# dayae1204/WeCLIP-ViT-CoMer

Measured on AMD Instinct MI355X. Metric: images/sec (train fwd+bwd) ViT-B/16 512x512 VOC, higher is better.
Workload: dtype f16 MFMA operands / f32 accumulate, f32 residual+softmax+LN, PAR f32 arithmetic on 16-bit fixed-point affinities (precision=fast); 1 GPU; WeCLIP VOC full train step (the reference's model: frozen CLIP ViT-B/16 + adapters + decoder + GradCAM/affinity/PAR pseudo-labels), batch 16/GPU at 512x512, K=2 classes/image (BASELINE configs[2] without the ViT-CoMer inserts, for which the reference has no code); global_batch=16, parallelism=dp1

## Files before the change

weclip-vit-comer_amd/csrc/affinity.hip:

```cpp
#include "common.h"

#define MAXK 4

struct MapPtrs {
    const float* p[12];
};

__global__ __launch_bounds__(256) void aff_weight_kernel(MapPtrs maps, int nmaps, const float* __restrict__ wgt,
                                                          const float* __restrict__ seg, float* __restrict__ W,
                                                          int L) {
    const int hw = L - 1;
    const int j = blockIdx.x * 256 + threadIdx.x, i = blockIdx.y, b = blockIdx.z;
    if (j >= hw) return;
    const long src = (long)b * L * L + (long)(i + 1) * L + (j + 1);
    float v[12];
#pragma unroll
    for (int l = 0; l < 12; ++l) v[l] = l < nmaps ? maps.p[l][src] : 0.f;
    float s = 0.f;
#pragma unroll
    for (int l = 0; l < 12; ++l)
        if (l < nmaps) s = fmaf(wgt[b * nmaps + l], v[l], s);
    const long dst = ((long)b * hw + i) * hw + j;
    if (seg) s *= seg[dst];
    W[dst] = s;
// ... 249 lines not shown
                    a += w[r][ch].x * cx[ch][0][k] + w[r][ch].y * cx[ch][1][k] + w[r][ch].z * cx[ch][2][k] + w[r][ch].w * cx[ch][3][k];
                p[r][k] = wave_sum(a);
            }
        if (lane == 0) {
#pragma unroll
            for (int r = 0; r < AF_RG; ++r)
#pragma unroll
                for (int k = 0; k < K; ++k) red[buf][wave][r][k] = p[r][k];
        }
        __syncthreads();
#pragma unroll
        for (int r = 0; r < AF_RG; ++r) {
            const int i = ig + r;
            if (i >= i1) continue;
            float rv[K];
#pragma unroll
            for (int k = 0; k < K; ++k) {
                const float dot = red[buf][0][r][k] + red[buf][1][r][k] + red[buf][2][r][k] + red[buf][3][r][k];
                if (MODE == 2) {
                    const float ri = rix[r];
                    if (tid == 0) y1[((long)b * hw + i) * K + k] = ri * dot;
                    rv[k] = ri * xix[r][k];
                } else {
                    rv[k] = 1.0f / dot;
                    if (tid == 0) rout[(long)b * hw + i] = rv[k];
                }
            }
            if (MODE != 1) {
#pragma unroll
                for (int ch = 0; ch < AF_MAXCH; ++ch)
#pragma unroll
                    for (int k = 0; k < K; ++k) {
                        ca[ch][0][k] = fmaf(w[r][ch].x, rv[k], ca[ch][0][k]);
                        ca[ch][1][k] = fmaf(w[r][ch].y, rv[k], ca[ch][1][k]);
                        ca[ch][2][k] = fmaf(w[r][ch].z, rv[k], ca[ch][2][k]);
                        ca[ch][3][k] = fmaf(w[r][ch].w, rv[k], ca[ch][3][k]);
                    }
            }
        }
    }
    if (MODE != 1) {
#pragma unroll
        for (int ch = 0; ch < AF_MAXCH; ++ch) {
            if (!okc[ch]) continue;
            const int j = ch * 1024 + tid * 4;
#pragma unroll
            for (int q = 0; q < 4; ++q)
#pragma unroll
                for (int k = 0; k < K; ++k) colpart[(((long)b * nblk + blk) * hw + j + q) * K + k] = ca[ch][q][k];
        }
    }
}

__global__ __launch_bounds__(256) void aff_colreduce_kernel(const float* __restrict__ colpart, const float* __restrict__ y1,
                                                             const float* __restrict__ c, float* __restrict__ out, int hw,
                                                             int K, int nblk, int mode) {
    const int e = blockIdx.x * 256 + threadIdx.x, b = blockIdx.y;
    if (e >= hw * K) return;
    const float* cp = colpart + (long)b * nblk * hw * K + e;
    const long st = (long)hw * K;
    float s = 0.f;
    int blk = 0;
    for (; blk + 8 <= nblk; blk += 8) {
        float v[8];
#pragma unroll
        for (int u = 0; u < 8; ++u) v[u] = cp[(blk + u) * st];
        s += ((v[0] + v[1]) + (v[2] + v[3])) + ((v[4] + v[5]) + (v[6] + v[7]));
    }
    for (; blk < nblk; ++blk) s += cp[blk * st];
    if (mode == 0) out[(long)b * hw + e] = 1.0f / s;
    else out[(long)b * hw * K + e] = 0.5f * (y1[(long)b * hw * K + e] + c[(long)b * hw + e / K] * s);
}

__global__ __launch_bounds__(256) void tsym_kernel(const float* __restrict__ W, const float* __restrict__ r,
                                                    const float* __restrict__ c, float* __restrict__ T, int hw) {
    const int j = blockIdx.x * 256 + threadIdx.x, i = blockIdx.y, b = blockIdx.z;
    if (j >= hw) return;
    const float* Wb = W + (long)b * hw * hw;
    const float* rb = r + (long)b * hw;
    const float* cb = c + (long)b * hw;
    T[((long)b * hw + i) * hw + j] = 0.5f * (rb[i] * Wb[(long)i * hw + j] * cb[j] + cb[i] * Wb[(long)j * hw + i] * rb[j]);
}

__global__ __launch_bounds__(256) void box_mask_kernel(const float* __restrict__ cam, const int* __restrict__ pair_img,
                                                        const int* __restrict__ pair_slot, float* __restrict__ V,
                                                        float* __restrict__ mask_out, int* __restrict__ boxes,
                                                        int* __restrict__ nbox, int maxbox, int h, int w, int K,
                                                        double thr) {
    extern __shared__ int smi[];
    const int hw = h * w, p = blockIdx.x, tid = threadIdx.x;
    int* lab = smi;
    int* xmin = lab + hw;
    int* xmax = xmin + hw;
    int* ymin = xmax + hw;
    int* ymax = ymin + hw;
    int* roots = ymax + hw;
    int* misc = roots + hw;
    const float* cp = cam + (long)p * hw;
    if (tid == 0) { misc[0] = 0; misc[2] = 0; }
    __syncthreads();
    int mx = 0;
    for (int i = tid; i < hw; i += 256) {
        const int u = (int)(unsigned char)(cp[i] * 255.0f);
        mx = u > mx ? u : mx;
    }
    atomicMax(&misc[0], mx);
    __syncthreads();
    const int theta = (int)(thr * (double)misc[0]);
    for (int i = tid; i < hw; i += 256) {
        const int u = (int)(unsigned char)(cp[i] * 255.0f);
        lab[i] = (u > theta) ? i : -1;
        xmin[i] = w; xmax[i] = -1; ymin[i] = h; ymax[i] = -1;
    }
    __syncthreads();
    for (int it = 0; it < hw + 2; ++it) {
        if (tid == 0) misc[1] = 0;
        __syncthreads();
        int changed = 0;
        for (int i = tid; i < hw; i += 256) {
            int l = lab[i];
            if (l < 0) continue;
            const int y = i / w, x = i - y * w;
            int best = l;
            for (int dy = -1; dy <= 1; ++dy)
                for (int dx = -1; dx <= 1; ++dx) {
                    const int yy = y + dy, xx = x + dx;
                    if (yy < 0 || yy >= h || xx < 0 || xx >= w) continue;
                    const int nl = lab[yy * w + xx];
                    if (nl >= 0 && nl < best) best = nl;
                }
            if (best < l) { lab[i] = best; changed = 1; }
        }
        if (changed) misc[1] = 1;
        __syncthreads();
        if (misc[1] == 0) break;
        for (int i = tid; i < hw; i += 256) {
            const int l = lab[i];
            if (l >= 0) {
                const int ll = lab[l];
                if (ll < l) lab[i] = ll;
            }
        }
        __syncthreads();
    }
    for (int i = tid; i < hw; i += 256) {
        int l = lab[i];
        if (l < 0) continue;
        while (lab[l] != l) l = lab[l];
        const int y = i / w, x = i - y * w;
        atomicMin(&xmin[l], x); atomicMax(&xmax[l], x);
        atomicMin(&ymin[l], y); atomicMax(&ymax[l], y);
    }
    __syncthreads();
    for (int i = tid; i < hw; i += 256)
        if (lab[i] == i) roots[atomicAdd(&misc[2], 1)] = i;
    __syncthreads();
    const int nroot = misc[2];
    if (boxes) {
        if (tid == 0) nbox[p] = nroot;
        for (int k = tid; k < nroot && k < maxbox; k += 256) {
            const int r = roots[k];
            int* bx = boxes + ((long)p * maxbox + k) * 4;
            bx[0] = xmin[r]; bx[1] = ymin[r];
            bx[2] = (xmax[r] + 1 < w - 1) ? xmax[r] + 1 : w - 1;
            bx[3] = (ymax[r] + 1 < h - 1) ? ymax[r] + 1 : h - 1;
        }
    }
    const int img = pair_img[p], slot = pair_slot[p];
    for (int i = tid; i < hw; i += 256) {
        const int y = i / w, x = i - y * w;
        int inside = 0;
        for (int k = 0; k < nroot && !inside; ++k) {
            const int r = roots[k];
            const int x0 = xmin[r], y0 = ymin[r];
            int x1 = xmax[r] + 1, y1 = ymax[r] + 1;
            x1 = x1 < w - 1 ? x1 : w - 1;
            y1 = y1 < h - 1 ? y1 : h - 1;
            inside = (x >= x0 && x < x1 && y >= y0 && y < y1);
        }
        if (mask_out) mask_out[(long)p * hw + i] = inside ? 1.f : 0.f;
        if (slot >= 0) V[((long)img * hw + i) * K + slot] = inside ? cp[i] : 0.f;
    }
}

__global__ __launch_bounds__(256) void refined_minmax_kernel(const float* __restrict__ R, float* __restrict__ stats,
                                                              int hw, int K) {
    __shared__ float red[16];
    const int k = blockIdx.x, b = blockIdx.y;
    float mn = INFINITY, mx = -INFINITY;
    for (int i = threadIdx.x; i < hw; i += 256) {
        const float v = R[((long)b * hw + i) * K + k];
        mn = fminf(mn, v);
        mx = fmaxf(mx, v);
    }
    mn = block_min(mn, red);
    mx = block_max(mx, red);
    if (threadIdx.x == 0) {
        stats[((long)b * K + k) * 2] = mn;
        stats[((long)b * K + k) * 2 + 1] = mx - mn;
    }
}

__global__ __launch_bounds__(256) void cam_upsample_kernel(const float* __restrict__ R, const float* __restrict__ stats,
                                                            const int* __restrict__ nk, float* __restrict__ cams,
                                                            int h, int w, int K, int C, int H, int W, float sy, float sx) {
    const int x = blockIdx.x * 64 + (threadIdx.x & 63), y = blockIdx.y * 4 + (threadIdx.x >> 6), b = blockIdx.z;
    if (x >= W || y >= H) return;
    float fy = fmaxf(sy * (y + 0.5f) - 0.5f, 0.f), fx = fmaxf(sx * (x + 0.5f) - 0.5f, 0.f);
    int y0 = (int)fy, x0 = (int)fx;
    if (y0 > h - 1) y0 = h - 1;
    if (x0 > w - 1) x0 = w - 1;
    const int y1 = y0 + (y0 < h - 1 ? 1 : 0), x1 = x0 + (x0 < w - 1 ? 1 : 0);
    const float ly = fy - y0, lx = fx - x0, hy = 1.f - ly, hx = 1.f - lx;
    const long HW = (long)H * W;
    const int n = nk[b];
    float best = -INFINITY;
    const float* Rb = R + (long)b * h * w * K;
    for (int k = 0; k < n; ++k) {
        const float mn = stats[((long)b * K + k) * 2], den = 1e-7f + stats[((long)b * K + k) * 2 + 1];
        const float v00 = (Rb[((long)y0 * w + x0) * K + k] - mn) / den, v01 = (Rb[((long)y0 * w + x1) * K + k] - mn) / den;
        const float v10 = (Rb[((long)y1 * w + x0) * K + k] - mn) / den, v11 = (Rb[((long)y1 * w + x1) * K + k] - mn) / den;
        const float v = hy * (hx * v00 + lx * v01) + ly * (hx * v10 + lx * v11);
        cams[((long)b * C + 1 + k) * HW + (long)y * W + x] = v;
        best = fmaxf(best, v);
    }
    for (int k = n; k < C - 1; ++k) cams[((long)b * C + 1 + k) * HW + (long)y * W + x] = 0.f;
    cams[(long)b * C * HW + (long)y * W + x] = 1.0f - best;
}

extern "C" int wc_aff_weight(const float* const* h_maps, int nmaps, const float* wgt, const float* seg, float* W,
                             int B, int L, void* stream) {
    WC_CHECK_ARG(h_maps && nmaps >= 1 && nmaps <= 12 && wgt && W && B > 0 && L > 1, "wc_aff_weight: bad argument");
    MapPtrs mp;
    for (int i = 0; i < 12; ++i) mp.p[i] = i < nmaps ? h_maps[i] : nullptr;
    const int hw = L - 1;
    hipLaunchKernelGGL(aff_weight_kernel, dim3(wc_cdiv(hw, 256), hw, B), dim3(256), 0, (hipStream_t)stream, mp, nmaps,
                       wgt, seg, W, L);
    WC_LAUNCH_CHECK("aff_weight_kernel");
    return WC_OK;
}

extern "C" int wc_aff_seg_weights(const float* const* h_maps, int nmaps, float* rowsum, float* diff, float* wgt,
                                  int B, int L, void* stream) {
    WC_CHECK_ARG(h_maps && nmaps >= 1 && nmaps <= 12 && rowsum && diff && wgt && B > 0 && L > 1,
                 "wc_aff_seg_weights: bad argument");
    MapPtrs mp;
    for (int i = 0; i < 12; ++i) mp.p[i] = i < nmaps ? h_maps[i] : nullptr;
    hipStream_t st = (hipStream_t)stream;
    hipLaunchKernelGGL(aff_rowsum_kernel, dim3(L - 1, nmaps, B), dim3(256), 0, st, mp, nmaps, rowsum, L);
    WC_LAUNCH_CHECK("aff_rowsum_kernel");
    hipLaunchKernelGGL(aff_keep_kernel, dim3(B), dim3(64), 0, st, rowsum, diff, wgt, nmaps, L - 1);
    WC_LAUNCH_CHECK("aff_keep_kernel");
    return WC_OK;
}

extern "C" int wc_matvec(const float* W, const float* X, const float* sin, const float* sout, const float* add,
                         float* out, int B, int hw, int K, int transpose, int recip, float alpha, void* stream) {
    WC_CHECK_ARG(W && X && out && B > 0 && hw > 0 && K > 0 && B <= 65535, "wc_matvec: bad argument");
    WC_CHECK_ARG(out != X && out != sin, "wc_matvec: out must not alias an input vector");
    hipStream_t st = (hipStream_t)stream;
    for (int k0 = 0; k0 < K; k0 += MAXK) {
        if (transpose)
            hipLaunchKernelGGL(matvec_cols_kernel, dim3(wc_cdiv(hw, 64), B), dim3(64 * MVC_SLICES), 0, st, W, X, sin, sout, add,
                               out, hw, K, k0, recip, alpha);
        else
            hipLaunchKernelGGL(matvec_rows_kernel, dim3(wc_cdiv(hw, 4), B), dim3(256), 0, st, W, X, sin, sout, add,
                               out, hw, K, k0, recip, alpha);
        WC_LAUNCH_CHECK("matvec kernel");
    }
    return WC_OK;
}

static bool aff_fused_ok(int hw) { return hw % 4 == 0 && hw <= 1024 * AF_MAXCH && hw >= 4; }

extern "C" int wc_aff_fused_supported(int hw) { return aff_fused_ok(hw) ? 1 : 0; }

extern "C" int wc_aff_weight_c1(const float* const* h_maps, int nmaps, const float* wgt, const float* seg, float* W, float* c1,
                                float* ws, int B, int L, void* stream) {
    WC_CHECK_ARG(h_maps && nmaps >= 1 && nmaps <= 12 && wgt && W && c1 && ws && B > 0 && B <= 65535 && L > 1 && aff_fused_ok(L - 1),
                 "wc_aff_weight_c1: bad argument");
    MapPtrs mp;
    for (int i = 0; i < 12; ++i) mp.p[i] = i < nmaps ? h_maps[i] : nullptr;
    const int hw = L - 1, nblk = wc_cdiv(hw, AF_RPBW);
    hipStream_t st = (hipStream_t)stream;
    const int pr = wc_prof_begin(stream);
    hipLaunchKernelGGL(aff_weight_colpart_kernel, dim3(nblk, B), dim3(256), 0, st, mp, nmaps, wgt, seg, W, ws, L);
    wc_prof_end(pr, "aff_weight_colpart_kernel", (double)B * hw * hw * 4.0 * (nmaps + 1 + (seg ? 1 : 0)), stream);
    WC_LAUNCH_CHECK("aff_weight_colpart_kernel");
    hipLaunchKernelGGL(aff_colreduce_kernel, dim3(wc_cdiv(hw, 256), B), dim3(256), 0, st, ws, nullptr, nullptr, c1, hw, 1, nblk, 0);
    WC_LAUNCH_CHECK("aff_colreduce_kernel");
    return WC_OK;
}

extern "C" int wc_aff_sinkhorn_step(const float* W, const float* c, float* r, float* c_next, float* ws, int B, int hw,
                                    int last, void* stream) {
    WC_CHECK_ARG(W && c && r && ws && (last || c_next) && B > 0 && B <= 65535 && aff_fused_ok(hw), "wc_aff_sinkhorn_step: bad argument");
    const int nblk = wc_cdiv(hw, AF_RPB);
    hipStream_t st = (hipStream_t)stream;
    const int pr = wc_prof_begin(stream);
    if (last) hipLaunchKernelGGL((aff_sweep_kernel<1, 1>), dim3(nblk, B), dim3(256), 0, st, W, c, nullptr, nullptr, r, nullptr, ws, hw);
    else hipLaunchKernelGGL((aff_sweep_kernel<0, 1>), dim3(nblk, B), dim3(256), 0, st, W, c, nullptr, nullptr, r, nullptr, ws, hw);
    wc_prof_end(pr, "aff_sweep_kernel", (double)B * hw * hw * 4.0 * (last ? 1 : 2), stream);
    WC_LAUNCH_CHECK("aff_sweep_kernel");
    if (!last) {
        hipLaunchKernelGGL(aff_colreduce_kernel, dim3(wc_cdiv(hw, 256), B), dim3(256), 0, st, ws, nullptr, nullptr, c_next, hw, 1, nblk, 0);
        WC_LAUNCH_CHECK("aff_colreduce_kernel");
    }
    return WC_OK;
}

extern "C" int wc_aff_tsym_apply(const float* W, const float* r, const float* c, const float* X, float* out, float* y1,
                                 float* ws, int B, int hw, int K, void* stream) {
    WC_CHECK_ARG(W && r && c && X && out && y1 && ws && out != X && B > 0 && B <= 65535 && K >= 1 && K <= 4 && aff_fused_ok(hw),
                 "wc_aff_tsym_apply: bad argument (K <= 4)");
    const int nblk = wc_cdiv(hw, AF_RPB);
    hipStream_t st = (hipStream_t)stream;
    dim3 grid(nblk, B);
    const int pr = wc_prof_begin(stream);
    switch (K) {
        case 1: hipLaunchKernelGGL((aff_sweep_kernel<2, 1>), grid, dim3(256), 0, st, W, c, r, X, nullptr, y1, ws, hw); break;
        case 2: hipLaunchKernelGGL((aff_sweep_kernel<2, 2>), grid, dim3(256), 0, st, W, c, r, X, nullptr, y1, ws, hw); break;
        case 3: hipLaunchKernelGGL((aff_sweep_kernel<2, 3>), grid, dim3(256), 0, st, W, c, r, X, nullptr, y1, ws, hw); break;
        default: hipLaunchKernelGGL((aff_sweep_kernel<2, 4>), grid, dim3(256), 0, st, W, c, r, X, nullptr, y1, ws, hw); break;
    }
    wc_prof_end(pr, "aff_sweep_kernel", (double)B * hw * hw * 4.0 * 2, stream);
    WC_LAUNCH_CHECK("aff_sweep_kernel");
    hipLaunchKernelGGL(aff_colreduce_kernel, dim3(wc_cdiv(hw * K, 256), B), dim3(256), 0, st, ws, y1, c, out, hw, K, nblk, 1);
    WC_LAUNCH_CHECK("aff_colreduce_kernel");
    return WC_OK;
}

extern "C" int wc_tsym(const float* W, const float* r, const float* c, float* T, int B, int hw, void* stream) {
    WC_CHECK_ARG(W && r && c && T && B > 0 && hw > 0, "wc_tsym: bad argument");
    hipLaunchKernelGGL(tsym_kernel, dim3(wc_cdiv(hw, 256), hw, B), dim3(256), 0, (hipStream_t)stream, W, r, c, T, hw);
    WC_LAUNCH_CHECK("tsym_kernel");
    return WC_OK;
}

extern "C" int wc_box_mask(const float* cam, const int* pair_img, const int* pair_slot, float* V, float* mask_out,
                           int* boxes, int* nbox, int maxbox, int P, int h, int w, int K, double thr, void* stream) {
    WC_CHECK_ARG(cam && pair_img && pair_slot && V && P > 0 && h > 0 && w > 0 && K > 0, "wc_box_mask: bad argument");
    WC_CHECK_ARG(!boxes || (nbox && maxbox > 0), "wc_box_mask: boxes needs nbox and maxbox");
    const size_t sm = ((size_t)6 * h * w + 4) * sizeof(int);
    WC_CHECK_ARG(sm <= 160 * 1024, "wc_box_mask: CAM grid too large (h*w <= 6800)");
    hipLaunchKernelGGL(box_mask_kernel, dim3(P), dim3(256), sm, (hipStream_t)stream, cam, pair_img, pair_slot, V,
                       mask_out, boxes, nbox, maxbox, h, w, K, thr);
    WC_LAUNCH_CHECK("box_mask_kernel");
    return WC_OK;
}

extern "C" int wc_cam_upsample(const float* R, const int* nk, float* stats, float* cams, int B, int h, int w, int K,
                               int C, int H, int W, void* stream) {
    WC_CHECK_ARG(R && nk && stats && cams && B > 0 && h > 0 && w > 0 && K > 0 && C >= 2 && C <= K + 1 && H > 0 && W > 0,
                 "wc_cam_upsample: bad argument");
    hipStream_t st = (hipStream_t)stream;
    hipLaunchKernelGGL(refined_minmax_kernel, dim3(K, B), dim3(256), 0, st, R, stats, h * w, K);
    WC_LAUNCH_CHECK("refined_minmax_kernel");
    hipLaunchKernelGGL(cam_upsample_kernel, dim3(wc_cdiv(W, 64), wc_cdiv(H, 4), B), dim3(256), 0, st, R, stats, nk,
                       cams, h, w, K, C, H, W, (float)h / H, (float)w / W);
    WC_LAUNCH_CHECK("cam_upsample_kernel");
    return WC_OK;
}
```

weclip-vit-comer_amd/csrc/gradcam.hip:

```cpp
#include "common.h"

typedef _Float16 f16x8 __attribute__((ext_vector_type(8)));
typedef float f32x16 __attribute__((ext_vector_type(16)));

#define LNP_ROWS 16
template <int NV>
__global__ __launch_bounds__(256) void lnpost_pool_kernel(const float* __restrict__ x2,
                                                           const float* __restrict__ w,
                                                           const float* __restrict__ bb, float eps,
                                                           float* __restrict__ partial, int L, int E,
                                                           int nchunk) {
    extern __shared__ float sm[];
    const int b = blockIdx.y, chunk = blockIdx.x, lane = threadIdx.x & 63, wv = threadIdx.x >> 6;
    float acc[NV], wv_[NV], bv[NV];
#pragma unroll
    for (int i = 0; i < NV; ++i) {
        const int e = lane + 64 * i;
        acc[i] = 0.f;
        wv_[i] = e < E ? w[e] : 0.f;
        bv[i] = e < E ? bb[e] : 0.f;
    }
    const int l0 = chunk * LNP_ROWS;
    for (int l = l0 + wv; l < l0 + LNP_ROWS && l < L; l += 4) {
        if (l == 0) continue;
        const float* xr = x2 + ((long)b * L + l) * E;
        float xv[NV];
        float s = 0.f;
#pragma unroll
        for (int i = 0; i < NV; ++i) {
            const int e = lane + 64 * i;
            xv[i] = e < E ? xr[e] : 0.f;
            s += xv[i];
        }
        const float mean = wave_sum(s) / E;
        float q = 0.f;
#pragma unroll
        for (int i = 0; i < NV; ++i) {
            const float d = (lane + 64 * i < E) ? xv[i] - mean : 0.f;
            q += d * d;
        }
        const float rstd = rsqrtf(wave_sum(q) / E + eps);
#pragma unroll
        for (int i = 0; i < NV; ++i)
            if (lane + 64 * i < E) acc[i] += (xv[i] - mean) * rstd * wv_[i] + bv[i];
    }
#pragma unroll
    for (int i = 0; i < NV; ++i)
        if (lane + 64 * i < E) sm[wv * E + lane + 64 * i] = acc[i];
    __syncthreads();
    for (int e = threadIdx.x; e < E; e += 256)
        partial[((long)b * nchunk + chunk) * E + e] = sm[e] + sm[E + e] + sm[2 * E + e] + sm[3 * E + e];
}

__global__ __launch_bounds__(512) void cam_head_kernel(const float* __restrict__ partial,
                                                        const float* __restrict__ proj,
                                                        const float* __restrict__ text,
                                                        const int* __restrict__ text_idx,
                                                        const int* __restrict__ n_text,
                                                        const int* __restrict__ pair_img,
                                                        const int* __restrict__ pair_cls, float logit_scale,
                                                        float* __restrict__ probs, float* __restrict__ df,
                                                        int L, int E, int Ed, int nchunk, int Tmax) {
    extern __shared__ float sm[];
    float* f = sm;
    float* y = f + E;
    float* dy = y + Ed;
    float* lg = dy + Ed;
    float* red = lg + Tmax;
    const int p = blockIdx.x, img = pair_img[p], cls = pair_cls[p], T = n_text[p], tid = threadIdx.x;
    for (int e = tid; e < E; e += 512) {
        const float* pp = partial + (long)img * nchunk * E + e;
        float s[8] = {0.f, 0.f, 0.f, 0.f, 0.f, 0.f, 0.f, 0.f};
        int c = 0;
        for (; c + 8 <= nchunk; c += 8)
#pragma unroll
            for (int u = 0; u < 8; ++u) s[u] += pp[(long)(c + u) * E];
        for (; c < nchunk; ++c) s[0] += pp[(long)c * E];
        f[e] = (((s[0] + s[1]) + (s[2] + s[3])) + ((s[4] + s[5]) + (s[6] + s[7]))) / (L - 1);
    }
    __syncthreads();
    for (int t = tid; t < Ed; t += 512) {
        float s0 = 0.f, s1 = 0.f, s2 = 0.f, s3 = 0.f;
        int e = 0;
        for (; e + 16 <= E; e += 16) {
            float pv[16];
#pragma unroll
            for (int u = 0; u < 16; ++u) pv[u] = proj[(long)(e + u) * Ed + t];
#pragma unroll
            for (int u = 0; u < 16; u += 4) {
                s0 = fmaf(f[e + u], pv[u], s0);
                s1 = fmaf(f[e + u + 1], pv[u + 1], s1);
                s2 = fmaf(f[e + u + 2], pv[u + 2], s2);
                s3 = fmaf(f[e + u + 3], pv[u + 3], s3);
            }
        }
        for (; e < E; ++e) s0 = fmaf(f[e], proj[(long)e * Ed + t], s0);
        y[t] = (s0 + s1) + (s2 + s3);
    }
    __syncthreads();
    float q = 0.f;
    for (int t = tid; t < Ed; t += 512) q += y[t] * y[t];
    const float ynorm = sqrtf(block_sum(q, red));
    __syncthreads();
    for (int t = tid; t < Ed; t += 512) y[t] /= ynorm;
    __syncthreads();
    const int lane = tid & 63, wv = tid >> 6;
    for (int t = wv; t < T; t += 8) {
        const float* tr = text + (long)text_idx[(long)p * Tmax + t] * Ed;
        float s = 0.f;
        for (int k = lane; k < Ed; k += 64) s += y[k] * tr[k];
        s = wave_sum(s);
        if (lane == 0) lg[t] = logit_scale * s;
    }
    __syncthreads();
    float mx = -INFINITY;
    for (int t = 0; t < T; ++t) mx = fmaxf(mx, lg[t]);
    float den = 0.f;
    for (int t = 0; t < T; ++t) den += expf(lg[t] - mx);
    __syncthreads();
    if (tid < T) {
        const float pr = expf(lg[tid] - mx) / den;
        probs[(long)p * Tmax + tid] = pr;
        lg[tid] = pr;
    }
    __syncthreads();
    const float pj = lg[cls];
    for (int k = tid; k < Ed; k += 512) {
        float s = 0.f;
        for (int t = 0; t < T; ++t) {
            const float dl = pj * ((t == cls ? 1.f : 0.f) - lg[t]);
            s = fmaf(dl, text[(long)text_idx[(long)p * Tmax + t] * Ed + k], s);
        }
        dy[k] = logit_scale * s;
    }
    __syncthreads();
    float dot = 0.f;
    for (int k = tid; k < Ed; k += 512) dot += y[k] * dy[k];
    dot = block_sum(dot, red);
    __syncthreads();
    for (int k = tid; k < Ed; k += 512) dy[k] = (dy[k] - y[k] * dot) / ynorm;
    __syncthreads();
    if ((Ed & 3) == 0) {
        const int rsub = lane >> 3, j = lane & 7;
        for (int e0 = wv * 8; e0 < E; e0 += 64) {
            const int e = e0 + rsub;
            float s = 0.f;
            if (e < E) {
                const float* pr = proj + (long)e * Ed;
#pragma unroll 4
                for (int k = 4 * j; k < Ed; k += 32) {
                    const float4 pv = *reinterpret_cast<const float4*>(pr + k);
                    s = fmaf(pv.x, dy[k], s);
                    s = fmaf(pv.y, dy[k + 1], s);
                    s = fmaf(pv.z, dy[k + 2], s);
                    s = fmaf(pv.w, dy[k + 3], s);
                }
            }
            s += __shfl_xor(s, 1, 64);
            s += __shfl_xor(s, 2, 64);
            s += __shfl_xor(s, 4, 64);
            if (j == 0 && e < E) df[(long)p * E + e] = s;
        }
    } else {
        for (int e = tid; e < E; e += 512) {
            const float* pr = proj + (long)e * Ed;
            float s = 0.f;
            for (int k = 0; k < Ed; ++k) s = fmaf(pr[k], dy[k], s);
            df[(long)p * E + e] = s;
        }
    }
}

template <int NV>
__global__ __launch_bounds__(256) void lnpost_bwd_kernel(const float* __restrict__ df,
                                                          const float* __restrict__ x2,
                                                          const float* __restrict__ w, float eps, float gs,
                                                          const int* __restrict__ pair_img,
                                                          float* __restrict__ d32, __half* __restrict__ dhi,
                                                          __half* __restrict__ dlo, int L, int E, long rows) {
    const long row = (long)blockIdx.x * 4 + (threadIdx.x >> 6);
    if (row >= rows) return;
    const int lane = threadIdx.x & 63;
    const int p = row / L, l = row % L;
    const long o = row * E;
    if (l == 0) {
        for (int e = lane; e < E; e += 64) {
            d32[o + e] = 0.f;
            dhi[o + e] = __float2half(0.f);
            if (dlo) dlo[o + e] = __float2half(0.f);
        }
        return;
    }
    const float* xr = x2 + ((long)pair_img[p] * L + l) * E;
    const float* g0 = df + (long)p * E;
    const float invn = 1.0f / (L - 1);
    if constexpr (NV > 0) {
        float xv[NV], gv[NV];
        float s = 0.f;
#pragma unroll
        for (int i = 0; i < NV; ++i) {
            const int e = lane + 64 * i, ec = e < E ? e : 0;
            const float ok = e < E ? 1.f : 0.f;
            xv[i] = xr[ec] * ok;
            gv[i] = g0[ec] * invn * w[ec] * ok;
            s += xv[i];
        }
        const float mean = wave_sum(s) / E;
        float q = 0.f;
#pragma unroll
        for (int i = 0; i < NV; ++i) {
            const float d = (lane + 64 * i < E) ? xv[i] - mean : 0.f;
            q += d * d;
        }
        const float rstd = rsqrtf(wave_sum(q) / E + eps);
        float sg = 0.f, sgx = 0.f;
#pragma unroll
        for (int i = 0; i < NV; ++i) {
            sg += gv[i];
            sgx += gv[i] * (xv[i] - mean) * rstd;
        }
        sg = wave_sum(sg) / E;
        sgx = wave_sum(sgx) / E;
#pragma unroll
        for (int i = 0; i < NV; ++i) {
            const int e = lane + 64 * i;
            if (e < E) {
                const float v = gs * rstd * (gv[i] - sg - (xv[i] - mean) * rstd * sgx);
                d32[o + e] = v;
                const __half h = __float2half(v);
                dhi[o + e] = h;
                if (dlo) dlo[o + e] = __float2half(v - __half2float(h));
            }
        }
    } else {
        float s = 0.f;
        for (int e = lane; e < E; e += 64) s += xr[e];
        const float mean = wave_sum(s) / E;
        float q = 0.f;
// ... 338 lines not shown
        const f16x8 kv = *reinterpret_cast<const f16x8*>(row + E);
        const f16x8 qv = *reinterpret_cast<const f16x8*>(row);
        const f16x8 dv = *reinterpret_cast<const f16x8*>(dob + (long)l * E);
        const float a = ub[l], s0 = sb[l], om = 1.0f - pb[l];
#pragma unroll
        for (int j = 0; j < 8; ++j) {
            cq[j] = fmaf(a, (float)kv[j], cq[j]);
            ck[j] = fmaf(s0, (float)qv[j], ck[j]);
            cv[j] = fmaf(om, (float)dv[j], cv[j]);
        }
    }
#pragma unroll
    for (int j = 0; j < 8; ++j) {
        red[0][sl][ch * 8 + j] = cq[j];
        red[1][sl][ch * 8 + j] = ck[j];
        red[2][sl][ch * 8 + j] = cv[j];
    }
    __syncthreads();
    const int d = threadIdx.x & 63, w3 = threadIdx.x >> 6;
    if (w3 < 3 && d < DH) {
        float t = 0.f;
        for (int k = 0; k < nsl; ++k) t += red[w3][k][d];
        float* out = c + (long)p * 3 * E + h * DH + d;
        if (w3 == 0) out[0] = t * inv_sqrt_dh;
        else if (w3 == 1) out[E] = -t * inv_qscale;
        else out[2 * E] = t;
    }
}

__global__ __launch_bounds__(1024) void cam_raw_kernel(const float* __restrict__ a32, const float* __restrict__ w,
                                                        const int* __restrict__ pair_img, float* __restrict__ cam, int L,
                                                        int E) {
    const int p = blockIdx.y, img = pair_img[p], lane = threadIdx.x & 63, wv = threadIdx.x >> 6;
    const int l = blockIdx.x * 16 + wv, hw = L - 1;
    if (l >= hw) return;
    const float* ar = a32 + ((long)img * L + l + 1) * E;
    const float* wr = w + (long)p * E;
    float s = 0.f;
    for (int e = lane; e < E; e += 64) s = fmaf(wr[e], ar[e], s);
    s = wave_sum(s);
    if (lane == 0) cam[(long)p * hw + l] = fmaxf(s, 0.f);
}

__global__ __launch_bounds__(1024) void cam_norm_kernel(float* __restrict__ cam, int hw) {
    extern __shared__ float sm[];
    float* cs = sm;
    float* red = cs + hw;
    const int p = blockIdx.x, tid = threadIdx.x;
    for (int l = tid; l < hw; l += 1024) cs[l] = cam[(long)p * hw + l];
    __syncthreads();
#pragma unroll 1
    for (int pass = 0; pass < 2; ++pass) {
        float mn = INFINITY;
        for (int l = tid; l < hw; l += 1024) mn = fminf(mn, cs[l]);
        mn = block_min(mn, red);
        float mx = -INFINITY;
        for (int l = tid; l < hw; l += 1024) mx = fmaxf(mx, cs[l] - mn);
        mx = block_max(mx, red);
        __syncthreads();
        for (int l = tid; l < hw; l += 1024) cs[l] = fmaxf((cs[l] - mn) / (1e-7f + mx), 0.f);
        __syncthreads();
    }
    for (int l = tid; l < hw; l += 1024) cam[(long)p * hw + l] = cs[l];
}

extern "C" int wc_cam_head(const float* x2, const float* lnw, const float* lnb, const float* proj,
                           const float* text, const int* text_idx, const int* n_text, const int* pair_img,
                           const int* pair_cls, float logit_scale, float* partial, float* probs, float* df,
                           int B, int P, int L, int E, int Ed, int Tmax, void* stream) {
    WC_CHECK_ARG(x2 && lnw && lnb && proj && text && text_idx && n_text && pair_img && pair_cls && partial &&
                     probs && df && B > 0 && P > 0 && L > 1 && E > 0 && Ed > 0,
                 "wc_cam_head: bad argument");
    WC_CHECK_ARG(Tmax > 0 && Tmax <= 512 && E <= 4096 && Ed <= 4096, "wc_cam_head: Tmax <= 512, E, Ed <= 4096");
    hipStream_t st = (hipStream_t)stream;
    const int nchunk = wc_cdiv(L, LNP_ROWS);
    WC_CHECK_ARG(E <= 1024, "wc_cam_head: E <= 1024");
    if (E <= 256)
        hipLaunchKernelGGL(lnpost_pool_kernel<4>, dim3(nchunk, B), dim3(256), 4 * E * sizeof(float), st, x2, lnw, lnb,
                           1e-5f, partial, L, E, nchunk);
    else
        hipLaunchKernelGGL(lnpost_pool_kernel<16>, dim3(nchunk, B), dim3(256), 4 * E * sizeof(float), st, x2, lnw, lnb,
                           1e-5f, partial, L, E, nchunk);
    WC_LAUNCH_CHECK("lnpost_pool_kernel");
    const size_t sm = (E + 2 * Ed + Tmax + 16) * sizeof(float);
    hipLaunchKernelGGL(cam_head_kernel, dim3(P), dim3(512), sm, st, partial, proj, text, text_idx, n_text,
                       pair_img, pair_cls, logit_scale, probs, df, L, E, Ed, nchunk, Tmax);
    WC_LAUNCH_CHECK("cam_head_kernel");
    return WC_OK;
}

extern "C" int wc_lnpost_bwd(const float* df, const float* x2, const float* lnw, float gs,
                             const int* pair_img, float* d32, void* dhi, void* dlo, int P, int L, int E,
                             void* stream) {
    WC_CHECK_ARG(df && x2 && lnw && pair_img && d32 && dhi && P > 0 && L > 1 && E > 0,
                 "wc_lnpost_bwd: bad argument");
    const long rows = (long)P * L;
#define LNPOST_BWD(NV_)                                                                                            \
    hipLaunchKernelGGL(lnpost_bwd_kernel<NV_>, dim3(wc_cdiv(rows, 4)), dim3(256), 0, (hipStream_t)stream, df, x2, \
                       lnw, 1e-5f, gs, pair_img, d32, (__half*)dhi, (__half*)dlo, L, E, rows)
    if (E <= 256) LNPOST_BWD(4);
    else if (E <= 768) LNPOST_BWD(12);
    else if (E <= 1024) LNPOST_BWD(16);
    else LNPOST_BWD(0);
#undef LNPOST_BWD
    WC_LAUNCH_CHECK("lnpost_bwd_kernel");
    return WC_OK;
}

extern "C" int wc_ln2_bwd_add(const float* da2, const float* dx2, const float* x1, const float* lnw, float gs,
                              const int* pair_img, void* g16, int P, int L, int E, void* stream) {
    WC_CHECK_ARG(da2 && dx2 && x1 && lnw && pair_img && g16 && P > 0 && L > 0 && E > 0 && gs > 0,
                 "wc_ln2_bwd_add: bad argument");
    const long rows = (long)P * L;
    WC_CHECK_ARG(E <= 1024, "wc_ln2_bwd_add: E <= 1024");
    if (E <= 256)
        hipLaunchKernelGGL(ln2_bwd_add_kernel<4>, dim3(wc_cdiv(rows, 4)), dim3(256), 0, (hipStream_t)stream, da2,
                           dx2, x1, lnw, 1e-5f, 1.0f / gs, pair_img, (__half*)g16, L, E, rows);
    else if (E <= 768)
        hipLaunchKernelGGL(ln2_bwd_add_kernel<12>, dim3(wc_cdiv(rows, 4)), dim3(256), 0, (hipStream_t)stream, da2,
                           dx2, x1, lnw, 1e-5f, 1.0f / gs, pair_img, (__half*)g16, L, E, rows);
    else
        hipLaunchKernelGGL(ln2_bwd_add_kernel<16>, dim3(wc_cdiv(rows, 4)), dim3(256), 0, (hipStream_t)stream, da2,
                           dx2, x1, lnw, 1e-5f, 1.0f / gs, pair_img, (__half*)g16, L, E, rows);
    WC_LAUNCH_CHECK("ln2_bwd_add_kernel");
    return WC_OK;
}

extern "C" int wc_attn_bwd_colsum(const void* qkv, const void* dO, const float* o32, const float* lse,
                                  const int* pair_img, float* delta, float* u, float* dS0, float* P0,
                                  float* c, int P, int L, int H, int DH, void* stream) {
    WC_CHECK_ARG(qkv && dO && o32 && lse && pair_img && delta && u && dS0 && P0 && c && P > 0 && L > 0 && H > 0,
                 "wc_attn_bwd_colsum: bad argument");
    WC_CHECK_ARG(DH == 64 || DH == 32, "wc_attn_bwd_colsum: head dim must be 32 or 64");
    WC_CHECK_ARG(P <= 65535 && H <= 65535, "wc_attn_bwd_colsum: too many pairs/heads for one launch");
    WC_CHECK_ARG(((uintptr_t)qkv | (uintptr_t)dO | (uintptr_t)o32) % 16 == 0, "wc_attn_bwd_colsum: operands must be 16-byte aligned");
    hipStream_t st = (hipStream_t)stream;
    const int E = H * DH;
    const long total = (long)P * L;
    hipLaunchKernelGGL(attn_delta_kernel, dim3(wc_cdiv(total, 4)), dim3(256), 0, st, (const __half*)dO, o32,
                       pair_img, delta, L, H, DH, total);
    WC_LAUNCH_CHECK("attn_delta_kernel");
    const int rr = L % 128;
    const int origin = (L >= 128 && rr > 0 && rr <= 8) ? rr : 0;
    const int nkt = wc_cdiv(L - origin, 128), PH = P * H;
    dim3 grid((unsigned)(nkt * ((PH + 7) / 8 * 8)));
    if (DH == 64) {
        const size_t lds = 2 * 128 * (64 * 2 + 16) + (2 * 128 * (64 * 2 + 16) + 1024) + 1024;
        hipLaunchKernelGGL(attn_bwd_colsum_kernel<64>, grid, dim3(256), lds, st, (const __half*)qkv,
                           (const __half*)dO, lse, delta, pair_img, u, dS0, P0, L, H, E, origin, nkt, PH);
        if (origin)
            hipLaunchKernelGGL(attn_bwd_colsum_edge_kernel<64>, dim3(H, P), dim3(256), 0, st, (const __half*)qkv,
                               (const __half*)dO, lse, delta, pair_img, u, dS0, P0, L, H, E, origin);
    } else {
        const size_t lds = 2 * 128 * (32 * 2 + 16) + (2 * 128 * (32 * 2 + 16) + 1024) + 1024;
        hipLaunchKernelGGL(attn_bwd_colsum_kernel<32>, grid, dim3(256), lds, st, (const __half*)qkv,
                           (const __half*)dO, lse, delta, pair_img, u, dS0, P0, L, H, E, origin, nkt, PH);
        if (origin)
            hipLaunchKernelGGL(attn_bwd_colsum_edge_kernel<32>, dim3(H, P), dim3(256), 0, st, (const __half*)qkv,
                               (const __half*)dO, lse, delta, pair_img, u, dS0, P0, L, H, E, origin);
    }
    WC_LAUNCH_CHECK("attn_bwd_colsum_kernel");
    hipLaunchKernelGGL(qkv_colsum_kernel, dim3(H, P), dim3(256), 0, st, (const __half*)qkv, (const __half*)dO, u,
                       dS0, P0, pair_img, c, L, H, DH, 1.0f / sqrtf((float)DH),
                       1.0f / 1.4426950408889634f);
    WC_LAUNCH_CHECK("qkv_colsum_kernel");
    return WC_OK;
}
// ... 77 lines not shown
```

weclip-vit-comer_amd/csrc/losses.hip:

```cpp
#include "common.h"

#define SEG_MAX_C 96

__device__ __forceinline__ void bil_index(int d, int in, float scale, int& i0, int& i1, float& l1) {
    float s = fmaxf(scale * (d + 0.5f) - 0.5f, 0.f);
    i0 = (int)s;
    if (i0 > in - 1) i0 = in - 1;
    i1 = i0 + (i0 < in - 1 ? 1 : 0);
    l1 = s - i0;
}

template <bool BWD>
__global__ __launch_bounds__(256) void seg_loss_kernel(const float* __restrict__ seg, const long* __restrict__ label,
                                                        float* __restrict__ part, const float* __restrict__ wts,
                                                        float* __restrict__ ghr, int nc, int h, int w, int H, int W,
                                                        float sy, float sx, int ignore) {
    __shared__ float red[16];
    const int x = blockIdx.x * 64 + (threadIdx.x & 63), y = blockIdx.y * 4 + (threadIdx.x >> 6), b = blockIdx.z;
    float nll = 0.f;
    int cls = -1;
    if (x < W && y < H) {
        const long lab = label[((long)b * H + y) * W + x];
        int y0, y1, x0, x1;
        float ly, lx;
// ... 311 lines not shown
                zc[c] = c < nc ? fmaf(ly, dv[c], av[c]) : -INFINITY;
                mx = fmaxf(mx, zc[c]);
                zl = c == lab ? zc[c] : zl;
            }
            float sum = 0.f;
#pragma unroll
            for (int c = 0; c < NCT; ++c) {
                zc[c] = c < nc ? __expf(zc[c] - mx) : 0.f;
                sum += zc[c];
            }
            const bool valid = lab != ignore && lab >= 0 && lab < nc;
            const float nll = mx + __logf(sum) - zl;
            if (valid && lab == 0) { l_bg += nll; c_bg += 1.f; }
            if (valid && lab != 0) { l_fg += nll; c_fg += 1.f; }
            const float wp = valid ? (lab == 0 ? wbg : wfg) : 0.f;
            const float u = wp / sum;
#pragma unroll
            for (int c = 0; c < NCT; ++c) {
                const float gval = fmaf(u, zc[c], c == lab ? -wp : 0.f);
                accT[c] += gval;
                accB[c] = fmaf(ly, gval, accB[c]);
            }
        }
#pragma unroll
        for (int c = 0; c < NCT; ++c)
            if (c < nc) {
                const long o = (((long)b * nc + c) * h) * W + x;
                if (y1s == ys) tmpA[o + (long)ys * W] = accT[c];
                else {
                    tmpA[o + (long)ys * W] = accT[c] - accB[c];
                    tmpB[o + (long)y1s * W] = accB[c];
                }
            }
    }
    const float a0 = block_sum(l_bg, red), a1 = block_sum(c_bg, red), a2 = block_sum(l_fg, red), a3 = block_sum(c_fg, red);
    if (threadIdx.x == 0) {
        const long blk = ((long)blockIdx.z * gridDim.y + blockIdx.y) * gridDim.x + blockIdx.x;
        part[blk * 4] = a0; part[blk * 4 + 1] = a1; part[blk * 4 + 2] = a2; part[blk * 4 + 3] = a3;
    }
}

template <bool SCALED>
__global__ __launch_bounds__(256) void seg_bwd_x2_kernel(const float* __restrict__ tmpA, const float* __restrict__ tmpB,
                                                          float* __restrict__ gsrc, long rows, int Hs, int Ws, int Wd, float sx,
                                                          const float* __restrict__ scale) {
    extern __shared__ float xrow[];
    const int lane = threadIdx.x & 63, wave = threadIdx.x >> 6;
    const long row = (long)blockIdx.x * 4 + wave;
    if (row >= rows) return;
    const int ys = (int)(row % Hs);
    float* v = xrow + wave * (Wd + (Wd >> 4) + 1);
    const float* TA = tmpA + row * Wd;
    const float* TB = tmpB + row * Wd;
    for (int x = lane; x < Wd; x += 64) v[x + (x >> 4)] = ys > 0 ? TA[x] + TB[x] : TA[x];
    asm volatile("s_waitcnt lgkmcnt(0)" ::: "memory");
    __builtin_amdgcn_wave_barrier();
    const float ix = 1.0f / sx;
    const float sc = SCALED ? scale[0] : 1.f;
    for (int xs = lane; xs < Ws; xs += 64) {
        int x_lo = (int)floorf((xs - 1.5f) * ix) - 1, x_hi = (int)ceilf((xs + 1.5f) * ix) + 1;
        if (x_lo < 0) x_lo = 0;
        if (x_hi > Wd - 1) x_hi = Wd - 1;
        float acc = 0.f;
        for (int x = x_lo; x <= x_hi; ++x) {
            int x0, x1;
            float lx;
            bil_index(x, Ws, sx, x0, x1, lx);
            const float wx = (x0 == xs ? 1.f - lx : 0.f) + (x1 == xs ? lx : 0.f);
            acc = fmaf(wx, v[x + (x >> 4)], acc);
        }
        gsrc[row * Ws + xs] = SCALED ? acc * sc : acc;
    }
}

extern "C" int wc_seg_loss_fwd_bwd(const float* seg, const int64_t* label, float* cnt, float* part, float* sums, float* tmp,
                                   float* grad, int B, int nc, int h, int w, int H, int W, int ignore, void* stream) {
    WC_CHECK_ARG(seg && label && cnt && part && sums && tmp && grad && B > 0 && B <= 65535 && nc > 0 && nc <= 24 &&
                 (long)B * nc <= 65535 && h > 0 && w > 0 && H >= h && W >= w, "wc_seg_loss_fwd_bwd: bad argument (nc <= 24)");
    hipStream_t st = (hipStream_t)stream;
    hipLaunchKernelGGL(seg_count_kernel, dim3(SEG_CNT_BLOCKS), dim3(256), 0, st, (const long*)label, cnt, (long)B * H * W, nc, ignore);
    WC_LAUNCH_CHECK("seg_count_kernel");
    dim3 grid(wc_cdiv(W, 64), wc_cdiv(h, 4), B);
    float* tmpB = tmp + (long)B * nc * h * W;
    hipLaunchKernelGGL(seg_loss_fused_kernel<24>, grid, dim3(256), 0, st, seg, (const long*)label, cnt, part, tmp, tmpB, nc, h, w, H,
                       W, (float)h / H, (float)w / W, ignore);
    WC_LAUNCH_CHECK("seg_loss_fused_kernel");
    hipLaunchKernelGGL(seg_loss_reduce_kernel, dim3(1), dim3(1024), 0, st, part, sums, (long)grid.x * grid.y * grid.z, 0);
    WC_LAUNCH_CHECK("seg_loss_reduce_kernel");
    const long rows = (long)B * nc * h;
    WC_CHECK_ARG(W <= 8192, "wc_seg_loss_fwd_bwd: W too large for the row buffer");
    hipLaunchKernelGGL(seg_bwd_x2_kernel<false>, dim3((unsigned)wc_cdiv(rows, 4)), dim3(256), 4 * (W + (W >> 4) + 1) * sizeof(float),
                       st, tmp, tmpB, grad, rows, h, w, W, (float)w / W, nullptr);
    WC_LAUNCH_CHECK("seg_bwd_x2_kernel");
    return WC_OK;
}

#define CE_MAX_C 128
#define CE_LSE_G 4
template <int CH, bool MULTI>
__global__ __launch_bounds__(256) void ce_loss_fused_kernel(const float* __restrict__ seg, const long* __restrict__ label,
                                                             float* __restrict__ part, float* __restrict__ tmpA,
                                                             float* __restrict__ tmpB, int nc, int nchunk, int h, int w, int H,
                                                             int W, float sy, float sx, int ignore) {
    __shared__ float red[16];
    const int x = blockIdx.x * 64 + (threadIdx.x & 63), ys = blockIdx.y * 4 + (threadIdx.x >> 6);
    const int b = blockIdx.z / nchunk, ck = blockIdx.z - b * nchunk, c0 = ck * CH;
    float l_sum = 0.f, n_ok = 0.f, n_bad = 0.f;
    if (x < W && ys < h) {
        int x0, x1;
        float lx;
        bil_index(x, w, sx, x0, x1, lx);
        const int y1s = ys + (ys < h - 1 ? 1 : 0);
        const float* S = seg + (long)b * nc * h * w;
        const long r0 = (long)ys * w, r1 = (long)y1s * w;
        float av[CH], dv[CH], accT[CH], accB[CH];
#pragma unroll
        for (int c = 0; c < CH; ++c) {
            accT[c] = accB[c] = 0.f;
            const float* Sc = S + (long)min(c0 + c, nc - 1) * h * w;
            const float a = (1.f - lx) * Sc[r0 + x0] + lx * Sc[r0 + x1];
            const float bb = (1.f - lx) * Sc[r1 + x0] + lx * Sc[r1 + x1];
            av[c] = a;
            dv[c] = bb - a;
        }
        const float iy = 1.0f / sy;
        int y_lo = ys == 0 ? 0 : (int)floorf((ys + 0.5f) * iy - 0.5f) - 1;
        int y_hi = ys == h - 1 ? H - 1 : (int)ceilf((ys + 1.5f) * iy - 0.5f) + 1;
        if (y_lo < 0) y_lo = 0;
        if (y_hi > H - 1) y_hi = H - 1;
        long labs[8];
        for (int y = y_lo; y <= y_hi; ++y) {
            if (((y - y_lo) & 7) == 0) {
#pragma unroll
                for (int u = 0; u < 8; ++u) labs[u] = label[((long)b * H + min(y + u, H - 1)) * W + x];
            }
            int y0, y1;
            float ly;
            bil_index(y, h, sy, y0, y1, ly);
            long lab = labs[0];
#pragma unroll
            for (int u = 1; u < 8; ++u) lab = ((y - y_lo) & 7) == u ? labs[u] : lab;
            if (y0 != ys) continue;
            float zc[CH];
            float mx = -INFINITY, sum = 0.f, zl = 0.f;
#pragma unroll
            for (int c = 0; c < CH; ++c) zc[c] = c0 + c < nc ? fmaf(ly, dv[c], av[c]) : -INFINITY;
            if constexpr (!MULTI) {
#pragma unroll
                for (int c = 0; c < CH; ++c) {
                    mx = fmaxf(mx, zc[c]);
                    zl = c == lab ? zc[c] : zl;
                }
            } else {
                for (int cb = 0; cb < nc; cb += CE_LSE_G) {
                    float zz[CE_LSE_G];
#pragma unroll
                    for (int u = 0; u < CE_LSE_G; ++u) {
                        const float* Sc = S + (long)min(cb + u, nc - 1) * h * w;
                        const float a = (1.f - lx) * Sc[r0 + x0] + lx * Sc[r0 + x1];
                        const float bb = (1.f - lx) * Sc[r1 + x0] + lx * Sc[r1 + x1];
                        zz[u] = cb + u < nc ? fmaf(ly, bb - a, a) : -INFINITY;
                    }
                    float m8 = mx;
#pragma unroll
                    for (int u = 0; u < CE_LSE_G; ++u) {
                        m8 = fmaxf(m8, zz[u]);
                        zl = cb + u == lab ? zz[u] : zl;
                    }
// ... 236 lines not shown
```

Before: 1276 images/sec.

## Speed up box mask, CAM head loops, and specialize seg loss for 21 classes

The box-mask kernel now runs with up to 1024 threads per block. It caches quantized CAM values in LDS, reduces the max with wave shuffles, and double-buffers the convergence flag to drop one barrier per iteration. The per-pixel loop over all box roots is replaced by a 2D difference-array prefix sum built with wave scans. The CAM head kernel caches text indices in shared memory and unrolls its projection and text loads more deeply to raise memory-level parallelism. The seg loss launches a template specialized for 21 classes. Together these add register pressure and complexity in several small pipeline kernels.

```diff
diff --git a/weclip-vit-comer_amd/csrc/affinity.hip b/weclip-vit-comer_amd/csrc/affinity.hip
--- a/weclip-vit-comer_amd/csrc/affinity.hip
+++ b/weclip-vit-comer_amd/csrc/affinity.hip
@@ -355,13 +355,13 @@
     T[((long)b * hw + i) * hw + j] = 0.5f * (rb[i] * Wb[(long)i * hw + j] * cb[j] + cb[i] * Wb[(long)j * hw + i] * rb[j]);
 }
 
-__global__ __launch_bounds__(256) void box_mask_kernel(const float* __restrict__ cam, const int* __restrict__ pair_img,
-                                                        const int* __restrict__ pair_slot, float* __restrict__ V,
-                                                        float* __restrict__ mask_out, int* __restrict__ boxes,
-                                                        int* __restrict__ nbox, int maxbox, int h, int w, int K,
-                                                        double thr) {
+__global__ __launch_bounds__(1024) void box_mask_kernel(const float* __restrict__ cam, const int* __restrict__ pair_img,
+                                                         const int* __restrict__ pair_slot, float* __restrict__ V,
+                                                         float* __restrict__ mask_out, int* __restrict__ boxes,
+                                                         int* __restrict__ nbox, int maxbox, int h, int w, int K,
+                                                         double thr) {
     extern __shared__ int smi[];
-    const int hw = h * w, p = blockIdx.x, tid = threadIdx.x;
+    const int hw = h * w, p = blockIdx.x, tid = threadIdx.x, nt = blockDim.x, lane = tid & 63, nwave = nt >> 6;
     int* lab = smi;
     int* xmin = lab + hw;
     int* xmax = xmin + hw;
@@ -370,27 +370,32 @@
     int* roots = ymax + hw;
     int* misc = roots + hw;
     const float* cp = cam + (long)p * hw;
-    if (tid == 0) { misc[0] = 0; misc[2] = 0; }
+    if (tid == 0) { misc[0] = 0; misc[2] = 0; misc[4] = 0; misc[5] = 0; }
     __syncthreads();
     int mx = 0;
-    for (int i = tid; i < hw; i += 256) {
+    for (int i = tid; i < hw; i += nt) {
         const int u = (int)(unsigned char)(cp[i] * 255.0f);
+        lab[i] = u;
         mx = u > mx ? u : mx;
     }
-    atomicMax(&misc[0], mx);
+#pragma unroll
+    for (int o = 32; o > 0; o >>= 1) {
+        const int t = __shfl_xor(mx, o, 64);
+        mx = t > mx ? t : mx;
+    }
+    if (lane == 0) atomicMax(&misc[0], mx);
     __syncthreads();
     const int theta = (int)(thr * (double)misc[0]);
-    for (int i = tid; i < hw; i += 256) {
-        const int u = (int)(unsigned char)(cp[i] * 255.0f);
-        lab[i] = (u > theta) ? i : -1;
+    for (int i = tid; i < hw; i += nt) {
+        lab[i] = (lab[i] > theta) ? i : -1;
         xmin[i] = w; xmax[i] = -1; ymin[i] = h; ymax[i] = -1;
     }
     __syncthreads();
     for (int it = 0; it < hw + 2; ++it) {
-        if (tid == 0) misc[1] = 0;
-        __syncthreads();
+        int* flag = misc + 4 + (it & 1);
+        if (tid == 0) misc[4 + ((it + 1) & 1)] = 0;
         int changed = 0;
-        for (int i = tid; i < hw; i += 256) {
+        for (int i = tid; i < hw; i += nt) {
             int l = lab[i];
             if (l < 0) continue;
             const int y = i / w, x = i - y * w;
@@ -404,10 +409,10 @@
                 }
             if (best < l) { lab[i] = best; changed = 1; }
         }
-        if (changed) misc[1] = 1;
+        if (changed) *flag = 1;
         __syncthreads();
-        if (misc[1] == 0) break;
-        for (int i = tid; i < hw; i += 256) {
+        if (*flag == 0) break;
+        for (int i = tid; i < hw; i += nt) {
             const int l = lab[i];
             if (l >= 0) {
                 const int ll = lab[l];
@@ -416,7 +421,7 @@
         }
         __syncthreads();
     }
-    for (int i = tid; i < hw; i += 256) {
+    for (int i = tid; i < hw; i += nt) {
         int l = lab[i];
         if (l < 0) continue;
         while (lab[l] != l) l = lab[l];
@@ -425,13 +430,13 @@
         atomicMin(&ymin[l], y); atomicMax(&ymax[l], y);
     }
     __syncthreads();
-    for (int i = tid; i < hw; i += 256)
+    for (int i = tid; i < hw; i += nt)
         if (lab[i] == i) roots[atomicAdd(&misc[2], 1)] = i;
     __syncthreads();
     const int nroot = misc[2];
     if (boxes) {
         if (tid == 0) nbox[p] = nroot;
-        for (int k = tid; k < nroot && k < maxbox; k += 256) {
+        for (int k = tid; k < nroot && k < maxbox; k += nt) {
             const int r = roots[k];
             int* bx = boxes + ((long)p * maxbox + k) * 4;
             bx[0] = xmin[r]; bx[1] = ymin[r];
@@ -439,18 +444,50 @@
             bx[3] = (ymax[r] + 1 < h - 1) ? ymax[r] + 1 : h - 1;
         }
     }
+    int* cover = lab;
+    for (int i = tid; i < hw; i += nt) cover[i] = 0;
+    __syncthreads();
+    for (int k = tid; k < nroot; k += nt) {
+        const int r = roots[k];
+        const int x0 = xmin[r], y0 = ymin[r];
+        int x1 = xmax[r] + 1, y1 = ymax[r] + 1;
+        x1 = x1 < w - 1 ? x1 : w - 1;
+        y1 = y1 < h - 1 ? y1 : h - 1;
+        if (x1 > x0 && y1 > y0) {
+            atomicAdd(&cover[y0 * w + x0], 1);
+            atomicAdd(&cover[y0 * w + x1], -1);
+            atomicAdd(&cover[y1 * w + x0], -1);
+            atomicAdd(&cover[y1 * w + x1], 1);
+        }
+    }
+    __syncthreads();
+    for (int y = tid >> 6; y < h; y += nwave) {
+        int carry = 0;
+        for (int xb = 0; xb < w; xb += 64) {
+            const int x = xb + lane;
+            int v = x < w ? cover[y * w + x] : 0;
+#pragma unroll
+            for (int o = 1; o < 64; o <<= 1) {
+                const int t = __shfl_up(v, o, 64);
+                if (lane >= o) v += t;
+            }
+            v += carry;
+            if (x < w) cover[y * w + x] = v;
+            carry = __shfl(v, 63, 64);
+        }
+    }
+    __syncthreads();
+    for (int x = tid; x < w; x += nt) {
+        int acc = 0;
+        for (int y = 0; y < h; ++y) {
+            acc += cover[y * w + x];
+            cover[y * w + x] = acc;
+        }
+    }
+    __syncthreads();
     const int img = pair_img[p], slot = pair_slot[p];
-    for (int i = tid; i < hw; i += 256) {
-        const int y = i / w, x = i - y * w;
-        int inside = 0;
-        for (int k = 0; k < nroot && !inside; ++k) {
-            const int r = roots[k];
-            const int x0 = xmin[r], y0 = ymin[r];
-            int x1 = xmax[r] + 1, y1 = ymax[r] + 1;
-            x1 = x1 < w - 1 ? x1 : w - 1;
-            y1 = y1 < h - 1 ? y1 : h - 1;
-            inside = (x >= x0 && x < x1 && y >= y0 && y < y1);
-        }
+    for (int i = tid; i < hw; i += nt) {
+        const bool inside = cover[i] > 0;
         if (mask_out) mask_out[(long)p * hw + i] = inside ? 1.f : 0.f;
         if (slot >= 0) V[((long)img * hw + i) * K + slot] = inside ? cp[i] : 0.f;
     }
@@ -614,9 +651,10 @@
                            int* boxes, int* nbox, int maxbox, int P, int h, int w, int K, double thr, void* stream) {
     WC_CHECK_ARG(cam && pair_img && pair_slot && V && P > 0 && h > 0 && w > 0 && K > 0, "wc_box_mask: bad argument");
     WC_CHECK_ARG(!boxes || (nbox && maxbox > 0), "wc_box_mask: boxes needs nbox and maxbox");
-    const size_t sm = ((size_t)6 * h * w + 4) * sizeof(int);
+    const size_t sm = ((size_t)6 * h * w + 8) * sizeof(int);
     WC_CHECK_ARG(sm <= 160 * 1024, "wc_box_mask: CAM grid too large (h*w <= 6800)");
-    hipLaunchKernelGGL(box_mask_kernel, dim3(P), dim3(256), sm, (hipStream_t)stream, cam, pair_img, pair_slot, V,
+    const int nt = h * w >= 1024 ? 1024 : (h * w <= 256 ? 256 : (h * w + 63) / 64 * 64);
+    hipLaunchKernelGGL(box_mask_kernel, dim3(P), dim3(nt), sm, (hipStream_t)stream, cam, pair_img, pair_slot, V,
                        mask_out, boxes, nbox, maxbox, h, w, K, thr);
     WC_LAUNCH_CHECK("box_mask_kernel");
     return WC_OK;
diff --git a/weclip-vit-comer_amd/csrc/gradcam.hip b/weclip-vit-comer_amd/csrc/gradcam.hip
--- a/weclip-vit-comer_amd/csrc/gradcam.hip
+++ b/weclip-vit-comer_amd/csrc/gradcam.hip
@@ -67,7 +67,9 @@
     float* dy = y + Ed;
     float* lg = dy + Ed;
     float* red = lg + Tmax;
+    int* tix = reinterpret_cast<int*>(red + 16);
     const int p = blockIdx.x, img = pair_img[p], cls = pair_cls[p], T = n_text[p], tid = threadIdx.x;
+    for (int t = tid; t < T; t += 512) tix[t] = text_idx[(long)p * Tmax + t];
     for (int e = tid; e < E; e += 512) {
         const float* pp = partial + (long)img * nchunk * E + e;
         float s[8] = {0.f, 0.f, 0.f, 0.f, 0.f, 0.f, 0.f, 0.f};
@@ -82,6 +84,18 @@
     for (int t = tid; t < Ed; t += 512) {
         float s0 = 0.f, s1 = 0.f, s2 = 0.f, s3 = 0.f;
         int e = 0;
+        for (; e + 48 <= E; e += 48) {
+            float pv[48];
+#pragma unroll
+            for (int u = 0; u < 48; ++u) pv[u] = proj[(long)(e + u) * Ed + t];
+#pragma unroll
+            for (int u = 0; u < 48; u += 4) {
+                s0 = fmaf(f[e + u], pv[u], s0);
+                s1 = fmaf(f[e + u + 1], pv[u + 1], s1);
+                s2 = fmaf(f[e + u + 2], pv[u + 2], s2);
+                s3 = fmaf(f[e + u + 3], pv[u + 3], s3);
+            }
+        }
         for (; e + 16 <= E; e += 16) {
             float pv[16];
 #pragma unroll
@@ -106,7 +120,7 @@
     __syncthreads();
     const int lane = tid & 63, wv = tid >> 6;
     for (int t = wv; t < T; t += 8) {
-        const float* tr = text + (long)text_idx[(long)p * Tmax + t] * Ed;
+        const float* tr = text + (long)tix[t] * Ed;
         float s = 0.f;
         for (int k = lane; k < Ed; k += 64) s += y[k] * tr[k];
         s = wave_sum(s);
@@ -127,9 +141,15 @@
     const float pj = lg[cls];
     for (int k = tid; k < Ed; k += 512) {
         float s = 0.f;
-        for (int t = 0; t < T; ++t) {
-            const float dl = pj * ((t == cls ? 1.f : 0.f) - lg[t]);
-            s = fmaf(dl, text[(long)text_idx[(long)p * Tmax + t] * Ed + k], s);
+        for (int t0 = 0; t0 < T; t0 += 8) {
+            float tv[8];
+#pragma unroll
+            for (int u = 0; u < 8; ++u) tv[u] = text[(long)tix[min(t0 + u, T - 1)] * Ed + k];
+#pragma unroll
+            for (int u = 0; u < 8; ++u) {
+                const int t = t0 + u;
+                if (t < T) s = fmaf(pj * ((t == cls ? 1.f : 0.f) - lg[t]), tv[u], s);
+            }
         }
         dy[k] = logit_scale * s;
     }
@@ -145,15 +165,20 @@
         for (int e0 = wv * 8; e0 < E; e0 += 64) {
             const int e = e0 + rsub;
             float s = 0.f;
-            if (e < E) {
-                const float* pr = proj + (long)e * Ed;
-#pragma unroll 4
-                for (int k = 4 * j; k < Ed; k += 32) {
-                    const float4 pv = *reinterpret_cast<const float4*>(pr + k);
-                    s = fmaf(pv.x, dy[k], s);
-                    s = fmaf(pv.y, dy[k + 1], s);
-                    s = fmaf(pv.z, dy[k + 2], s);
-                    s = fmaf(pv.w, dy[k + 3], s);
+            const float* pr = proj + (long)min(e, E - 1) * Ed;
+            for (int kb = 4 * j; kb < Ed; kb += 512) {
+                float4 pv[16];
+#pragma unroll
+                for (int u = 0; u < 16; ++u) pv[u] = *reinterpret_cast<const float4*>(pr + (kb + 32 * u < Ed ? kb + 32 * u : 0));
+#pragma unroll
+                for (int u = 0; u < 16; ++u) {
+                    const int k = kb + 32 * u;
+                    if (k < Ed) {
+                        s = fmaf(pv[u].x, dy[k], s);
+                        s = fmaf(pv[u].y, dy[k + 1], s);
+                        s = fmaf(pv[u].z, dy[k + 2], s);
+                        s = fmaf(pv[u].w, dy[k + 3], s);
+                    }
                 }
             }
             s += __shfl_xor(s, 1, 64);
@@ -658,7 +683,7 @@
         hipLaunchKernelGGL(lnpost_pool_kernel<16>, dim3(nchunk, B), dim3(256), 4 * E * sizeof(float), st, x2, lnw, lnb,
                            1e-5f, partial, L, E, nchunk);
     WC_LAUNCH_CHECK("lnpost_pool_kernel");
-    const size_t sm = (E + 2 * Ed + Tmax + 16) * sizeof(float);
+    const size_t sm = (E + 2 * Ed + 2 * Tmax + 16) * sizeof(float);
     hipLaunchKernelGGL(cam_head_kernel, dim3(P), dim3(512), sm, st, partial, proj, text, text_idx, n_text,
                        pair_img, pair_cls, logit_scale, probs, df, L, E, Ed, nchunk, Tmax);
     WC_LAUNCH_CHECK("cam_head_kernel");
diff --git a/weclip-vit-comer_amd/csrc/losses.hip b/weclip-vit-comer_amd/csrc/losses.hip
--- a/weclip-vit-comer_amd/csrc/losses.hip
+++ b/weclip-vit-comer_amd/csrc/losses.hip
@@ -417,8 +417,12 @@
     WC_LAUNCH_CHECK("seg_count_kernel");
     dim3 grid(wc_cdiv(W, 64), wc_cdiv(h, 4), B);
     float* tmpB = tmp + (long)B * nc * h * W;
-    hipLaunchKernelGGL(seg_loss_fused_kernel<24>, grid, dim3(256), 0, st, seg, (const long*)label, cnt, part, tmp, tmpB, nc, h, w, H,
-                       W, (float)h / H, (float)w / W, ignore);
+    if (nc == 21)
+        hipLaunchKernelGGL(seg_loss_fused_kernel<21>, grid, dim3(256), 0, st, seg, (const long*)label, cnt, part, tmp, tmpB, nc, h, w,
+                           H, W, (float)h / H, (float)w / W, ignore);
+    else
+        hipLaunchKernelGGL(seg_loss_fused_kernel<24>, grid, dim3(256), 0, st, seg, (const long*)label, cnt, part, tmp, tmpB, nc, h, w,
+                           H, W, (float)h / H, (float)w / W, ignore);
     WC_LAUNCH_CHECK("seg_loss_fused_kernel");
     hipLaunchKernelGGL(seg_loss_reduce_kernel, dim3(1), dim3(1024), 0, st, part, sums, (long)grid.x * grid.y * grid.z, 0);
     WC_LAUNCH_CHECK("seg_loss_reduce_kernel");
```

Measured after the change: 1289 images/sec, median of 6. +1.1%, better.
